# achiever04/face-recognition-platform

Measured on AMD Instinct MI355X. Metric: faces/sec (detect+embed+match) on 1080p @ 100k gallery, higher is better.
Workload: dtype f16; 1 GPU; 32x1080x1920 BGR frames per GPU per step resident in HBM, host results out every step, 2 batches in flight per GPU (one handle = one stream each, used round-robin), forced K=10 faces/frame, 100000-identity fp16 gallery, FRPDet detector fp16 + ArcFace IResNet-100 fp16 (synthetic seeded weights); batch_frames=32, faces_per_frame=10, gallery=100000, streams=1, lanes=2, lane_warmup_steps=20

## Files before the change

### face-recognition-platform_amd/csrc/aux_kernels.hip

```cpp
#include <hip/hip_runtime.h>
#include <stdint.h>
#include "frp_internal.h"

namespace frp {

typedef _Float16 half8 __attribute__((ext_vector_type(8)));

__global__ __launch_bounds__(256) void preprocess_kernel(const uint8_t* __restrict__ src, int B, int H, int W,
                                                         long row_stride, long frame_stride,
                                                         _Float16* __restrict__ out, int Hc, int Wc, int rgb_in) {
    const long total = (long)B * Hc * Wc;
    for (long i = (long)blockIdx.x * blockDim.x + threadIdx.x; i < total; i += (long)gridDim.x * blockDim.x) {
        const int x = (int)(i % Wc);
        const long r = i / Wc;
        const int y = (int)(r % Hc);
        const int b = (int)(r / Hc);
        float c0 = 0.f, c1 = 0.f, c2 = 0.f;
        if (y < H && x < W) {
            const uint8_t* p = src + b * frame_stride + y * row_stride + 3L * x;
            c0 = (float)p[0]; c1 = (float)p[1]; c2 = (float)p[2];
        }
        const float r_ = rgb_in ? c0 : c2, g_ = c1, b_ = rgb_in ? c2 : c0;
        half8 v;
        v[0] = (_Float16)((r_ - 127.5f) * (1.0f / 128.0f));
// ... 299 lines not shown
    return hipGetLastError();
}

hipError_t launch_mfma_peak(const _Float16* src, float* dst, int blocks, int iters, hipStream_t stream) {
    hipLaunchKernelGGL(mfma_peak_kernel, dim3(blocks), dim3(256), 0, stream, src, dst, iters);
    return hipGetLastError();
}

hipError_t launch_fill_random_f16(_Float16* p, long n, unsigned seed, float scale, hipStream_t stream) {
    if (n <= 0) return hipSuccess;
    hipLaunchKernelGGL(fill_random_f16_kernel, dim3(4096), dim3(256), 0, stream, p, n, seed, scale);
    return hipGetLastError();
}
#endif

__global__ __launch_bounds__(256) void tensor_hash_kernel(const uint4* __restrict__ src, long n16, unsigned long long* __restrict__ slot) {
    unsigned long long acc = 0;
    for (long i = (long)blockIdx.x * blockDim.x + threadIdx.x; i < n16; i += (long)gridDim.x * blockDim.x) {
        const uint4 v = src[i];
        unsigned long long a = ((unsigned long long)v.x << 32 | v.y) ^ 0x9e3779b97f4a7c15ull * (unsigned long long)(i + 1);
        unsigned long long b = ((unsigned long long)v.z << 32 | v.w) + 0xc2b2ae3d27d4eb4full * (unsigned long long)(i + 1);
        a ^= a >> 29; a *= 0xbf58476d1ce4e5b9ull; a ^= a >> 32;
        b ^= b >> 31; b *= 0x94d049bb133111ebull; b ^= b >> 29;
        acc += a + (b << 1 | b >> 63);
    }
#pragma unroll
    for (int o = 32; o; o >>= 1) acc += __shfl_xor(acc, o);
    if ((threadIdx.x & 63) == 0) atomicAdd(slot, acc);
}
hipError_t launch_tensor_hash(const void* src, size_t bytes, unsigned long long* slot, hipStream_t stream) {
    const long n16 = (long)(bytes / 16);
    if (n16 <= 0) return hipSuccess;
    hipLaunchKernelGGL(tensor_hash_kernel, dim3(1024), dim3(256), 0, stream, (const uint4*)src, n16, slot);
    return hipGetLastError();
}

}
```

### face-recognition-platform_amd/csrc/frp_api.cpp

```cpp
#include <hip/hip_runtime.h>

#include <algorithm>
#include <cmath>
#include <cstdio>
#include <cstdlib>
#include <cstring>
#include <mutex>
#include <string>
#include <vector>
#include <thread>
#include <atomic>

#include "frp.h"
#include "frp_blob.h"
#include "frp_internal.h"
#include "frp_handle.h"
#include "jpeg_host.h"

using namespace frp;

#define FRP_WINO_MIN_FACES 128
Switches frp::read_switches() {
    auto set = [](const char* n) { return getenv(n) ? 1 : 0; };
    const char *sm = getenv("FRP_SMALL_M"), *wm = getenv("FRP_WINO_MIN_FACES");
    Switches s{};
    s.small_m = !sm ? 0 : (sm[0] == '0' ? -1 : 1);
    s.wino_min_faces = wm ? atoi(wm) : FRP_WINO_MIN_FACES;
    s.s2 = set("FRP_S2"); s.host_count = set("FRP_HOST_COUNT"); s.match_v1 = set("FRP_MATCH_V1");
    s.no_fused_stem12 = set("FRP_NO_FUSED_STEM12"); s.no_fused_stem = set("FRP_NO_FUSED_STEM");
    s.no_emb_stem = set("FRP_NO_EMB_STEM"); s.no_stem_fuse = set("FRP_NO_STEM_FUSE");
    s.no_wino = set("FRP_NO_WINO"); s.no_kconcat = set("FRP_NO_KCONCAT");
    return s;
}

const ProcessSwitches& frp::process_switches() {
    static const ProcessSwitches s = [] {
        const char* jh = getenv("FRP_JPEG_DEVICE_HUFFMAN");
        return ProcessSwitches{getenv("FRP_NO_GRAPH") != nullptr, getenv("FRP_C64_ALL") != nullptr, !jh ? 0 : (jh[0] == '0' ? -1 : 1)};
    }();
    return s;
// ... 1025 lines not shown
int frp_debug_det_hashes(frp_handle* h, int32_t enable, uint64_t* out64) {
    if (!h) return FRP_ERR_INVALID;
    Guard g(h);
    if (enable) {
        FRPCHK(ensure(h, h->det_hashes, 64 * 8));
        h->det_hash_on = true;
    } else h->det_hash_on = false;
    if (out64) {
        if (!h->det_hashes.p) return fail(h, FRP_ERR_INVALID, "hashes were never enabled");
        HIPCHK(h, hipMemcpyAsync(out64, h->det_hashes.p, 64 * 8, hipMemcpyDeviceToHost, h->stream));
        HIPCHK(h, hipStreamSynchronize(h->stream));
    }
    return FRP_OK;
}

int frp_debug_det_prefix(frp_handle* h, int32_t n_ops, void* out_f16, int64_t out_bytes, int32_t* th, int32_t* tw, int32_t* tc) {
    if (!h) return FRP_ERR_INVALID;
    Guard g(h);
    if (!h->have_weights) return fail(h, FRP_ERR_NO_WEIGHTS, "no weights loaded");
    if (h->rB <= 0) return fail(h, FRP_ERR_INVALID, "no resident frames (call frp_upload_frames)");
    if (n_ops <= 0 || n_ops > (int)h->det.ops.size()) return fail(h, FRP_ERR_INVALID, "op count out of range");
    const int B = h->rB, Hc = h->canvas_h, Wc = h->canvas_w;
    const Switches sw = read_switches();
    const bool fused = h->det.det_stem && !sw.no_fused_stem;
    if (!fused) return fail(h, FRP_ERR_INVALID, "prefix runs need the fused stem");
    if (n_ops == 1 && h->det.det_stem12 && (Hc % 4) == 0 && (Wc % 4) == 0 && !sw.no_fused_stem12)
        return fail(h, FRP_ERR_INVALID, "op 0 has no tensor while both stems run as one kernel: set FRP_NO_FUSED_STEM12 to read the stem1 map");
    FRPCHK(plan_net(h, h->det, B, Hc, Wc, fused));
    StemParams sp{};
    sp.frames = h->det_scaled ? (const uint8_t*)h->scaled.p : (const uint8_t*)h->frames.p;
// ... 279 lines not shown
```

### face-recognition-platform_amd/csrc/frp_internal.h

```cpp
#pragma once
#include <hip/hip_runtime.h>
#include <stdint.h>
#include <type_traits>

#define FRP_ACT_NONE 0
#define FRP_ACT_RELU 1
#define FRP_ACT_PRELU 2
#define FRP_FLAG_BORDER_BIAS 1
#define FRP_FLAG_OUT_F32 2
#define FRP_FLAG_RES_UP2 4
#define FRP_FLAG_FLATTEN 8
#define FRP_FLAG_F8 32
#define FRP_FLAG_OUT_FP8 64
#define FRP_CHIP_PIX (112 * 112)
#ifndef FRP_MAX_FACES_CAP
#define FRP_MAX_FACES_CAP 128
#endif

#include "jpeg_host.h"

namespace frp {

struct Switches {
    int small_m;
    int s2;
    int no_fused_stem12;
    int no_fused_stem;
    int no_emb_stem;
    int no_stem_fuse;
    int wino_min_faces;
    int host_count;
    int match_v1;
    int no_wino;
    int no_kconcat;
};
static_assert(std::has_unique_object_representations_v<Switches>, "run_net keys captured graphs by the bytes of a Switches");
Switches read_switches();

struct ProcessSwitches {
    bool no_graph;
    bool c64_all;
    int jpeg_device_huffman;
};
const ProcessSwitches& process_switches();

struct ConvParams {
    const _Float16* x;
    const _Float16* w;
    const float* bias;
// ... 148 lines not shown

struct JpegHuffParams {
    const uint8_t* scan;
    const uint32_t* int_off;
    const JpegHuffTableDev* tables;
    int16_t* coef;
    int32_t* err;
    long coef_per_image;
    int B, n_int, ri;
    int mcus_x, mcus_y, components;
    int hs[3], vs[3], bx[3];
    long comp_off[3];
};
hipError_t launch_jpeg_huffman(const JpegHuffParams& p, hipStream_t stream);

hipError_t launch_tensor_hash(const void* src, size_t bytes, unsigned long long* slot, hipStream_t stream);
hipError_t launch_resize_u8(const uint8_t* src, int B, int H, int W, uint8_t* dst, int Hs, int Ws, hipStream_t stream);

struct AlignParams {
    const uint8_t* frames;
    int B, H, W;
    long row_stride, frame_stride;
    const float* kps;
    const int32_t* counts;
    int max_faces;
    const int32_t* face_slot;
    int n_faces;
    int rgb_in;
    _Float16* chips;
    const int32_t* n_dev;
};
// ... 72 lines not shown
```

### face-recognition-platform_amd/csrc/net_program.cpp

```cpp
#include "net_program.h"

#include <algorithm>
#include <cmath>
#include <cstdio>
#include <cstring>

#include "frp_handle.h"

namespace frp {

static float fp8_e4m3_value(unsigned char c) {
    const int e = (c >> 3) & 0xF, m = c & 7;
    float v;
    if (e == 15 && m == 7) v = 0.f;
    else if (e == 0) v = std::ldexp((float)m / 8.0f, -6);
    else v = std::ldexp(1.0f + (float)m / 8.0f, e - 7);
    return (c & 0x80) ? -v : v;
}

uint16_t f32_to_f16_bits(float f) {
    uint32_t x;
    memcpy(&x, &f, 4);
    const uint32_t sign = (x >> 16) & 0x8000u;
    x &= 0x7fffffffu;
// ... 247 lines not shown
}

void analyse_net(Net& net) {
    const int n = (int)net.ops.size();
    net.det_stem = stem_fusable(net);
    net.det_stem12 = stem12_fusable(net);
    net.fc_op = n && (net.ops[n - 1].flags & FRP_FLAG_OUT_F32) ? n - 1 : -1;
    net.next_launch.assign(n, -1);
    for (int i = n - 1, nx = -1; i >= 0; --i) {
        net.next_launch[i] = nx;
        if (!net.kc_skip[i]) nx = i;
    }
    net.emb_stem = net.fuse_ok = net.fuse_even_only = false;
    net.fuse_op = -1;
    if (n) analyse_emb_stem(net);
}

}

int load_program(frp_handle* h, const frp_blob_header& hd, const unsigned char* blob, size_t bytes, const Switches& sw,
                 std::vector<unsigned char>& image) {
    Net &det = h->det, &emb = h->emb;
    det.is_det = true;
    FRPCHK(parse_net(h, blob, bytes, hd.det_ops_offset, hd.n_det_ops, hd.n_det_bufs, hd.det_in_buf, hd.det_in_ch, hd.data_bytes, det));
    FRPCHK(parse_net(h, blob, bytes, hd.emb_ops_offset, hd.n_emb_ops, hd.n_emb_bufs, hd.emb_in_buf, hd.emb_in_ch, hd.data_bytes, emb));
    for (int l = 0; l < 3; ++l)
        if (hd.det_head_buf[l] >= hd.n_det_bufs) return fail(h, FRP_ERR_BLOB, "head buffer id out of range");
    if (hd.emb_out_buf >= hd.n_emb_bufs) return fail(h, FRP_ERR_BLOB, "embedding buffer id out of range");
    image.assign(blob + hd.data_offset, blob + hd.data_offset + hd.data_bytes);
    for (Net* net : {&det, &emb}) {
        const size_t n_ops = net->ops.size();
        net->wino_off.assign(n_ops, -1);
// ... 47 lines not shown
    for (int i = 0; i < net.n_bufs; ++i)
        if (need[i]) FRPCHK(ensure(h, net.bufs[i], need[i]));
    return FRP_OK;
}

namespace {

struct Pass {
    frp_handle* h;
    const Switches& sw;
    Net& net;
    int batch, H, W;
    const StemParams* stem;
    const int32_t* n_dev;
    bool allow_wino;
    const char* weights() const { return (const char*)h->wdata.p; }
};

struct FusedStem {
    bool on = false;
    EmbStemParams p{};
};

int launched(frp_handle* h, hipError_t e, const char* what) {
    return e == hipSuccess ? FRP_OK : fail(h, FRP_ERR_HIP, std::string(what) + ": " + hipGetErrorString(e));
}

int run_det_stems(const Pass& ps, PassEffects& fx, size_t& next) {
    frp_handle* h = ps.h;
    const Net& net = ps.net;
    const StemParams& st = *ps.stem;
    const char* wbase = ps.weights();
    if (net.ops.empty()) return FRP_OK;
    const frp_conv_op& a = net.ops[0];
    if (net.det_stem12 && (st.Hc % 4) == 0 && (st.Wc % 4) == 0 && !ps.sw.no_fused_stem12) {
        const frp_conv_op& b = net.ops[1];
        Stem12Params sp{};
        sp.frames = st.frames; sp.B = st.B; sp.H = st.H; sp.W = st.W;
        sp.row_stride = st.row_stride; sp.frame_stride = st.frame_stride;
        sp.Hc = st.Hc; sp.Wc = st.Wc; sp.Ho1 = st.Hc / 2; sp.Wo1 = st.Wc / 2; sp.Ho2 = st.Hc / 4; sp.Wo2 = st.Wc / 4;
        sp.rgb_in = st.rgb_in;
        sp.w1 = (const _Float16*)(wbase + a.w_off); sp.bias1 = (const float*)(wbase + a.bias_off);
        sp.w2 = (const _Float16*)(wbase + b.w_off); sp.bias2 = (const float*)(wbase + b.bias_off);
        sp.out = (_Float16*)net.bufs[b.out_buf].p;
        FRPCHK(launched(h, launch_stem12_u8(sp, h->stream), "launch_stem12_u8"));
        fx.dims[a.out_buf] = {sp.Ho1, sp.Wo1, 32, false};
        fx.dims[b.out_buf] = {sp.Ho2, sp.Wo2, 64, false};
        fx.flops += 2.0 * ps.batch * sp.Ho1 * sp.Wo1 * 9.0 * 3 * 32 + 2.0 * ps.batch * sp.Ho2 * sp.Wo2 * 9.0 * 32 * 64;
        fx.launches += 1;
        next = 2;
        if (!h->det_hash_on) return FRP_OK;
        return launched(h, launch_tensor_hash(sp.out, (size_t)ps.batch * sp.Ho2 * sp.Wo2 * 64 * 2, (unsigned long long*)h->det_hashes.p + 1, h->stream),
                        "tensor_hash");
    }
    StemParams sp = st;
    sp.w = (const _Float16*)(wbase + a.w_off);
    sp.bias = (const float*)(wbase + a.bias_off);
    sp.out = (_Float16*)net.bufs[a.out_buf].p;
    FRPCHK(launched(h, launch_stem_u8(sp, h->stream), "launch_stem_u8"));
    fx.dims[a.out_buf] = {sp.Ho, sp.Wo, 32, false};
    fx.flops += 2.0 * ps.batch * sp.Ho * sp.Wo * 9.0 * 3 * 32;
    fx.launches += 1;
    next = 1;
    return FRP_OK;
}

int run_emb_stem(const Pass& ps, PassEffects& fx, size_t& next, FusedStem& fused) {
    const Net& net = ps.net;
    if (!net.emb_stem || ps.sw.no_emb_stem) return FRP_OK;
    const frp_conv_op& a = net.ops[0];
    const char* wbase = ps.weights();
    EmbStemParams ep{};
    ep.x = (const _Float16*)net.bufs[a.in_buf].p;
    ep.M = ps.batch; ep.H = ps.H; ep.W = ps.W;
    ep.w = (const _Float16*)(wbase + a.w_off);
    ep.bias = (const float*)(wbase + a.bias_off);
    ep.slope = (const float*)(wbase + a.slope_off);
    ep.out = (_Float16*)net.bufs[a.out_buf].p;
    ep.n_dev = ps.n_dev;
    fused.on = net.fuse_ok && !ps.sw.no_stem_fuse && ps.sw.small_m <= 0 && conv3x3_c64_fuses_stem(ps.batch, ps.H, ps.W, ps.h->n_cu);
    if (fused.on) {
        fused.p = ep;
    } else {
        FRPCHK(launched(ps.h, launch_emb_stem(ep, ps.h->stream), "launch_emb_stem"));
        fx.launches += 1;
    }
    fx.dims[a.out_buf] = {ps.H, ps.W, 64, false};
    fx.flops += 2.0 * ps.batch * ps.H * ps.W * 9.0 * 3 * 64;
    next = 1;
    return FRP_OK;
}

ConvParams conv_params_for(const Pass& ps, size_t i, const TensorDims& in, const std::vector<TensorDims>& d, const FusedStem& fused) {
// ... 27 lines not shown
        p.flags |= FRP_FLAG_F8;
        p.wscale = (const float*)(wbase + op.w_off + (welems + 15) / 16 * 16);
        p.in_scale = op.in_scale;
    }
    if (net.kc_src[i] >= 0) {
        const frp_conv_op& sc = net.ops[net.kc_src[i]];
        p.x2 = (const _Float16*)net.bufs[sc.in_buf].p;
        p.Cin2 = sc.cin;
        p.w = (const _Float16*)(wbase + net.kc_w_off[i]);
        p.bias = (const float*)(wbase + net.kc_bias_off[i]);
        p.res = nullptr;
    }
    if (op.flags & FRP_OPFLAG_OUT_FP8) p.flags |= FRP_FLAG_OUT_FP8;
    if (op.out2_buf >= 0) p.out2 = net.bufs[op.out2_buf].p;
    if ((op.flags & FRP_OPFLAG_OUT_FP8) || op.out2_buf >= 0) p.out_scale = op.out_scale;
    const int nx = net.next_launch[i];
    if (nx < 0) return p;
    const frp_conv_op& no = net.ops[nx];
    if (net.kc_src[nx] >= 0) {
        p.pf_ptr = wbase + net.kc_w_off[nx];
        p.pf_bytes = (unsigned)((size_t)no.cout * (9 * (size_t)no.cin + net.ops[net.kc_src[nx]].cin) * 2);
    } else if (ps.allow_wino && net.wino_off[nx] >= 0) {
        p.pf_ptr = wbase + net.wino_off[nx];
        p.pf_bytes = (unsigned)std::min<size_t>(conv3x3_wino_image_bytes(no.cin, no.cout), 0x7fffffffu);
    } else {
        const size_t es = (no.flags & FRP_OPFLAG_FP8_MFMA) ? 1 : 2;
        p.pf_ptr = wbase + no.w_off;
        p.pf_bytes = (unsigned)std::min<size_t>((size_t)no.cout * no.ksize * no.ksize * no.cin * es, 0x7fffffffu);
    }
    return p;
// ... 8 lines not shown
    p.ksplit = ps.n_dev ? -1 : ks;
    p.out = h->splitk_ws.p;
    fc.ksplit = p.ksplit;
    fc.bias = p.bias;
    fc.ktot = op.ksize * op.ksize * op.cin;
}

void charge(const frp_conv_op& op, const TensorDims& out, int batch, PassEffects& fx) {
    const int cin_r = op.real_ch & 0xffff, cout_r = (op.real_ch >> 16) & 0xffff;
    const double fl = 2.0 * batch * out.h * out.w * (double)op.ksize * op.ksize * (cin_r ? cin_r : op.cin) * (cout_r ? cout_r : op.cout);
    fx.flops += fl;
    fx.launches += 1;
    if (op.flags & FRP_OPFLAG_FP8_MFMA) { fx.f8_flops += fl; fx.f8_launches += 1; }
}

int walk(const Pass& ps, PassEffects& fx) {
    frp_handle* h = ps.h;
    const Net& net = ps.net;
    fx = PassEffects();
    std::vector<TensorDims>& d = fx.dims;
    d.assign(net.n_bufs, TensorDims());
    d[net.in_buf] = {ps.H, ps.W, net.in_ch, false};
    const bool hashing = net.is_det && h->det_hash_on;
    if (hashing) HIPCHK(h, hipMemsetAsync(h->det_hashes.p, 0, 64 * 8, h->stream));
    size_t i = 0;
    FusedStem fused;
    if (ps.stem) FRPCHK(run_det_stems(ps, fx, i));
    else FRPCHK(run_emb_stem(ps, fx, i, fused));
    size_t end = net.ops.size();
    if (net.is_det && h->det_op_limit >= 0) end = std::min(end, (size_t)h->det_op_limit);
    for (; i < end; ++i) {
        const frp_conv_op& op = net.ops[i];
        const TensorDims in = flat_input(d[op.in_buf], op), out = conv_out_dims(in, op);
        if (net.kc_skip[i]) {
            set_out_dims(d, op, out);
            fx.flops += 2.0 * ps.batch * out.h * out.w * (double)op.cin * op.cout;
            continue;
        }
        ConvParams p = conv_params_for(ps, i, in, d, fused);
        if ((int)i == net.fc_op) pick_fc_splitk(ps, op, in, out, p, fx.fc);
        FRPCHK(launched(h, launch_conv(p, h->stream), "launch_conv"));
        set_out_dims(d, op, out);
        if (hashing && i < 64 && !ps.n_dev)
            FRPCHK(launched(h, launch_tensor_hash(net.bufs[op.out_buf].p, (size_t)ps.batch * out.h * out.w * out.c * (out.f32 ? 4 : 2),
                                                  (unsigned long long*)h->det_hashes.p + i, h->stream), "tensor_hash"));
        charge(op, out, ps.batch, fx);
    }
    return FRP_OK;
}

std::string graph_key(const Pass& ps) {
    char kb[512];
    int len = snprintf(kb, sizeof kb, "%c|%d|%d|%d|%d|%p|%p|", ps.net.is_det ? 'd' : 'e', ps.batch, ps.H, ps.W, (int)ps.allow_wino, (const void*)ps.n_dev,
                       (const void*)ps.h->wdata.p);
    if (const StemParams* stem = ps.stem; stem && len > 0 && len < (int)sizeof kb)
        len += snprintf(kb + len, sizeof kb - len, "%p|%d|%d|%d|%ld|%ld|%d|%d|%d", (const void*)stem->frames, stem->B, stem->H, stem->W, stem->row_stride,
                        stem->frame_stride, stem->Hc, stem->Wc, stem->rgb_in);
    if (len <= 0 || len >= (int)sizeof kb) return std::string();
    return std::string(kb, len) + std::string(reinterpret_cast<const char*>(&ps.sw), sizeof ps.sw);
}

int launch_or_replay(const Pass& ps, PassEffects& fx) {
    frp_handle* h = ps.h;
    if (process_switches().no_graph || h->det_hash_on || h->det_op_limit >= 0) return walk(ps, fx);
    const std::string key = graph_key(ps);
    if (key.empty()) return walk(ps, fx);
    for (size_t i = 0; i < h->graphs.size(); ++i) {
        NetGraph& g = h->graphs[i];
        if (g.key != key) continue;
        if (g.epoch != h->alloc_epoch) {
            (void)hipGraphExecDestroy(g.exec);
            h->graphs.erase(h->graphs.begin() + i);
// ... 76 lines not shown
```

### face-recognition-platform_amd/csrc/net_program.h

```cpp
#pragma once
#include <string>
#include <vector>

#include "frp_blob.h"
#include "frp_internal.h"

struct frp_handle;

namespace frp {

struct DevBuf {
    void* p = nullptr;
    size_t cap = 0;
};

struct TensorDims {
    int h = 0, w = 0, c = 0;
    bool f32 = false;
    bool f8 = false;
};

struct Net {
    std::vector<frp_conv_op> ops;
    int n_bufs = 0;
// ... 1 lines not shown
    bool is_det = false;
    std::vector<DevBuf> bufs;
    std::vector<TensorDims> dims;
    std::vector<int64_t> wino_off;
    std::vector<int> kc_skip;
    std::vector<int> kc_src;
    std::vector<int64_t> kc_w_off, kc_bias_off;
    bool det_stem = false;
    bool det_stem12 = false;
    bool emb_stem = false;
    int fuse_op = -1;
    bool fuse_ok = false;
    bool fuse_even_only = false;
    int fc_op = -1;
    std::vector<int> next_launch;
};

struct FcSplitK {
    int ksplit = 0, ktot = 0;
    const float* bias = nullptr;
};

struct PassEffects {
    double flops = 0, f8_flops = 0;
    int64_t launches = 0, f8_launches = 0;
    FcSplitK fc;
    std::vector<TensorDims> dims;
};

struct NetGraph {
    std::string key;
// ... 21 lines not shown
```

### face-recognition-platform_amd/native.py

```python
from __future__ import annotations

import ctypes as C
import os
import threading
from typing import Optional, Sequence, Tuple

import numpy as np

_HERE = os.path.dirname(os.path.abspath(__file__))
os.environ.setdefault("GPU_MAX_HW_QUEUES", "8")

LIB_PATH = os.environ.get("FRP_LIB") or os.path.join(_HERE, "libfrp.so")

EMB_DIM = 512
CHIP = 112
MAX_FACES_CAP = 128
MAX_TOPK = 64
FLAG_FORCED_K, FLAG_RGB, FLAG_NO_MATCH, FLAG_WITHIN = 1, 2, 4, 8
F32, F16, F64 = 0, 1, 2
QUALITY_TILE_H, QUALITY_TILE_W = 32, 64

ABI_SYMBOLS = [
    "frp_create", "frp_destroy", "frp_last_error", "frp_version", "frp_load_weights",
    "frp_gallery_set", "frp_gallery_set_device", "frp_gallery_reserve", "frp_gallery_commit", "frp_gallery_cancel", "frp_gallery_device_ptr", "frp_gallery_update_row", "frp_gallery_remove_row",
    "frp_jpeg_info_get", "frp_jpeg_coefficients", "frp_upload_jpeg_async", "frp_debug_jpeg_device_batches", "frp_debug_graph_replays",
    "frp_dist_unique_id", "frp_dist_init", "frp_dist_destroy", "frp_gallery_allgather",
    "frp_gallery_size", "frp_gallery_get", "frp_gallery_exact", "frp_gallery_distances", "frp_gallery_get_exact",
    "frp_process_frames", "frp_upload_frames", "frp_process_resident", "frp_fetch_results", "frp_synchronize",
    "frp_host_alloc", "frp_host_free", "frp_upload_frames_async", "frp_swap_frames",
    "frp_detect", "frp_detect_resident", "frp_get_det_source", "frp_finish_faces", "frp_get_head_map", "frp_debug_det_prefix", "frp_debug_det_hashes", "frp_decode_heads", "frp_align", "frp_embed_aligned", "frp_embed_faces",
    "frp_match", "frp_match_scores", "frp_match_within", "frp_set_within", "frp_fetch_within", "frp_face_quality", "frp_conv2d_nhwc", "frp_conv2d_f8", "frp_get_counters", "frp_reset_counters", "frp_set_profile",
]


class FrpConfig(C.Structure):
    _fields_ = [("struct_size", C.c_int32), ("max_batch", C.c_int32), ("max_faces", C.c_int32),
                ("max_h", C.c_int32), ("max_w", C.c_int32), ("profile", C.c_int32), ("reserved", C.c_int32 * 10)]


class FrpCounters(C.Structure):
    _fields_ = [("struct_size", C.c_int32), ("calls", C.c_int32), ("frames", C.c_int64), ("faces", C.c_int64),
                ("ms_h2d", C.c_double), ("ms_preprocess", C.c_double), ("ms_det_conv", C.c_double),
                ("ms_decode", C.c_double), ("ms_align", C.c_double), ("ms_emb_conv", C.c_double),
                ("ms_l2norm", C.c_double), ("ms_match", C.c_double), ("ms_d2h", C.c_double), ("ms_total", C.c_double),
                ("det_conv_flops", C.c_double), ("emb_conv_flops", C.c_double),
# ... 35 lines not shown

def jpeg_coefficients(data: bytes):
    info = jpeg_info(data)
    if info is None:
        raise FrpError(-1, "not a baseline JPEG the decoder covers")
    n = sum(info["mcus_x"] * info["h_samp"][c] * info["mcus_y"] * info["v_samp"][c] * 64 for c in range(info["components"]))
    coef = np.zeros(n, np.int16)
    q = np.zeros((3, 64), np.uint16)
    ji = JpegInfo()
    ptr, keep = _byte_ptr(data)
    rc = load_library().frp_jpeg_coefficients(ptr, len(data), _ptr(coef), n, _ptr(q), C.byref(ji))
    del keep
    if rc != 0:
        raise FrpError(rc, "corrupt JPEG scan data")
    return info, coef, q


class FrpError(RuntimeError):
    def __init__(self, code: int, msg: str):
        super().__init__(f"frp error {code}: {msg}")
        self.code = code


_lib = None


def kernel_source_hash() -> str:
    import glob
    import hashlib
    h = hashlib.sha256()
# ... 53 lines not shown
    lib.frp_detect.argtypes = [vp, vp, i32, i32, i32, i64, i32, f32, f32, u32, vp, vp, vp, vp, vp]
    lib.frp_detect_resident.argtypes = [vp, i32, i32, i32, i32, f32, f32, u32, vp, vp, vp, vp, vp]
    lib.frp_get_det_source.argtypes = [vp, vp, i64, C.POINTER(i32), C.POINTER(i32)]
    lib.frp_finish_faces.argtypes = [vp, i32, vp, vp, vp, vp, i32, u32, vp, vp, vp]
    lib.frp_get_head_map.argtypes = [vp, i32, vp, i64, C.POINTER(i32), C.POINTER(i32)]
    lib.frp_debug_jpeg_device_batches.argtypes = [vp]
    lib.frp_debug_jpeg_device_batches.restype = C.c_int64
    lib.frp_debug_graph_replays.argtypes = [vp]
    lib.frp_debug_graph_replays.restype = C.c_int64
    lib.frp_dist_unique_id.argtypes = [vp]
    lib.frp_dist_init.argtypes = [vp, vp, i32, i32]
    lib.frp_dist_destroy.argtypes = [vp]
    lib.frp_gallery_allgather.argtypes = [vp, vp, i64, i32, i64]
    lib.frp_debug_det_prefix.argtypes = [vp, i32, vp, i64, C.POINTER(i32), C.POINTER(i32), C.POINTER(i32)]
    lib.frp_debug_det_hashes.argtypes = [vp, i32, vp]
    lib.frp_decode_heads.argtypes = [vp, vp, vp, vp, i32, i32, i32, i32, f32, f32, u32, vp, vp, vp, vp, vp]
    lib.frp_align.argtypes = [vp, vp, i32, i32, i64, vp, i32, u32, vp]
    lib.frp_embed_aligned.argtypes = [vp, vp, i32, vp]
    lib.frp_embed_faces.argtypes = [vp, vp, i32, i32, i64, vp, i32, u32, vp]
    lib.frp_match.argtypes = [vp, vp, i32, i32, vp, vp]
    lib.frp_match_scores.argtypes = [vp, vp, i32, vp, i64]
    if hasattr(lib, "frp_match_within"):
        lib.frp_match_within.argtypes = [vp, vp, i32, f32, i32, vp, vp, vp]
        lib.frp_set_within.argtypes = [vp, f32, i32]
        lib.frp_fetch_within.argtypes = [vp, i32, i32, i32, vp, vp, vp]
    if hasattr(lib, "frp_face_quality"):
        lib.frp_face_quality.argtypes = [vp, vp, i32, u32, vp]
    lib.frp_conv2d_nhwc.argtypes = [vp, vp, i32, i32, i32, i32, vp, i32, i32, i32, vp, vp, vp, i32, i32, i32, i32, vp]
    lib.frp_conv2d_f8.argtypes = [vp, vp, i32, i32, i32, i32, vp, i32, vp, vp, vp, vp, i32, i32, f32, f32, vp, vp]
    if hasattr(lib, "frp_kstep_lab"):
# ... 478 lines not shown
```

### include/frp.h

```cpp
#ifndef FRP_H
#define FRP_H

#include <stddef.h>
#include <stdint.h>

#ifdef __cplusplus
extern "C" {
#endif

#define FRP_EMB_DIM 512
#define FRP_CHIP 112
#define FRP_KPS 5
#define FRP_MAX_FACES_CAP 128
#define FRP_MAX_TOPK 64

typedef enum frp_status {
    FRP_OK = 0,
    FRP_ERR_INVALID = -1,
    FRP_ERR_HIP = -2,
    FRP_ERR_NO_WEIGHTS = -3,
    FRP_ERR_NO_GALLERY = -4,
    FRP_ERR_BLOB = -5,
    FRP_ERR_OOM = -6
} frp_status;
// ... 91 lines not shown
int frp_dist_destroy(frp_handle* h);
int frp_gallery_allgather(frp_handle* h, const void* shard, int64_t shard_rows, int32_t dtype, int64_t n_total);

int frp_detect(frp_handle* h, const uint8_t* bgr, int32_t B, int32_t H, int32_t W, int64_t row_stride,
               int32_t max_faces, float det_thresh, float nms_iou, uint32_t flags,
               float* boxes, float* kps, float* scores, int32_t* counts, int32_t* anchor_idx);
int frp_detect_resident(frp_handle* h, int32_t B, int32_t det_h, int32_t det_w, int32_t max_faces, float det_thresh, float nms_iou,
                        uint32_t flags, float* boxes, float* kps, float* scores, int32_t* counts, int32_t* anchor_idx);
int frp_get_det_source(frp_handle* h, uint8_t* out, int64_t out_bytes, int32_t* hs, int32_t* ws);
int frp_finish_faces(frp_handle* h, int32_t B, const float* boxes, const float* kps, const float* scores, const int32_t* counts,
                     int32_t max_faces, uint32_t flags, float* emb, int32_t* match_idx, float* match_cos);

int frp_get_head_map(frp_handle* h, int32_t level, void* out_f16, int64_t out_bytes, int32_t* hl, int32_t* wl);
int frp_debug_det_prefix(frp_handle* h, int32_t n_ops, void* out_f16, int64_t out_bytes, int32_t* th, int32_t* tw, int32_t* tc);
int frp_debug_det_hashes(frp_handle* h, int32_t enable, uint64_t* out64);
int frp_decode_heads(frp_handle* h, const void* head8, const void* head16, const void* head32,
                     int32_t B, int32_t canvas_h, int32_t canvas_w, int32_t max_faces, float det_thresh, float nms_iou,
                     uint32_t flags, float* boxes, float* kps, float* scores, int32_t* counts, int32_t* anchor_idx);
int frp_align(frp_handle* h, const uint8_t* bgr, int32_t H, int32_t W, int64_t row_stride,
              const float* kps, int32_t M, uint32_t flags, void* chips_f16);
int frp_embed_aligned(frp_handle* h, const uint8_t* chips, int32_t M, float* emb);
int frp_embed_faces(frp_handle* h, const uint8_t* bgr, int32_t H, int32_t W, int64_t row_stride,
                    const float* kps, int32_t M, uint32_t flags, float* emb);
int frp_match(frp_handle* h, const float* q, int32_t M, int32_t topk, int32_t* idx, float* cos);
int frp_match_scores(frp_handle* h, const float* q, int32_t M, float* cos_all, int64_t n_cols);
int frp_match_within(frp_handle* h, const float* q, int32_t M, float min_cos, int32_t cap, int32_t* idx, float* cos, int32_t* n_hits);

int frp_face_quality(frp_handle* h, const int32_t* rects, int32_t n, uint32_t flags, int64_t* sums);

int frp_conv2d_nhwc(frp_handle* h, const void* x, int32_t N, int32_t H, int32_t W, int32_t Cin,
// ... 17 lines not shown
```

Baseline: 27220 faces/s.

## Run front detector layers in frame groups so activations stay cache-resident

Finds the leading run of frame-local conv ops whose activation maps are large, then executes that run group-by-group over frames instead of layer-by-layer over the whole batch. The group size is chosen so live activations per group fit a byte budget (about the last-level cache size), with some preference for groups that fill the CUs evenly. The aim is to keep intermediate maps from spilling to HBM between layers. In exchange it issues more, smaller kernel launches with lower occupancy per launch, and the graph key now includes the plan. A hash offset parameter and a debug plan API are added.

New measurement: 26630 faces/s. 0.978x the previous value.

```diff
diff --git a/face-recognition-platform_amd/csrc/aux_kernels.hip b/face-recognition-platform_amd/csrc/aux_kernels.hip
--- a/face-recognition-platform_amd/csrc/aux_kernels.hip
+++ b/face-recognition-platform_amd/csrc/aux_kernels.hip
@@ -337,10 +337,11 @@
 }
 #endif
 
-__global__ __launch_bounds__(256) void tensor_hash_kernel(const uint4* __restrict__ src, long n16, unsigned long long* __restrict__ slot) {
+__global__ __launch_bounds__(256) void tensor_hash_kernel(const uint4* __restrict__ src, long n16, long first16, unsigned long long* __restrict__ slot) {
     unsigned long long acc = 0;
-    for (long i = (long)blockIdx.x * blockDim.x + threadIdx.x; i < n16; i += (long)gridDim.x * blockDim.x) {
-        const uint4 v = src[i];
+    for (long j = (long)blockIdx.x * blockDim.x + threadIdx.x; j < n16; j += (long)gridDim.x * blockDim.x) {
+        const uint4 v = src[j];
+        const long i = j + first16;
         unsigned long long a = ((unsigned long long)v.x << 32 | v.y) ^ 0x9e3779b97f4a7c15ull * (unsigned long long)(i + 1);
         unsigned long long b = ((unsigned long long)v.z << 32 | v.w) + 0xc2b2ae3d27d4eb4full * (unsigned long long)(i + 1);
         a ^= a >> 29; a *= 0xbf58476d1ce4e5b9ull; a ^= a >> 32;
@@ -351,11 +352,11 @@
     for (int o = 32; o; o >>= 1) acc += __shfl_xor(acc, o);
     if ((threadIdx.x & 63) == 0) atomicAdd(slot, acc);
 }
-hipError_t launch_tensor_hash(const void* src, size_t bytes, unsigned long long* slot, hipStream_t stream) {
+hipError_t launch_tensor_hash(const void* src, size_t bytes, unsigned long long* slot, hipStream_t stream, size_t first_byte) {
     const long n16 = (long)(bytes / 16);
     if (n16 <= 0) return hipSuccess;
-    hipLaunchKernelGGL(tensor_hash_kernel, dim3(1024), dim3(256), 0, stream, (const uint4*)src, n16, slot);
-    return hipGetLastError();
-}
-
-}
+    hipLaunchKernelGGL(tensor_hash_kernel, dim3(1024), dim3(256), 0, stream, (const uint4*)src, n16, (long)(first_byte / 16), slot);
+    return hipGetLastError();
+}
+
+}
diff --git a/face-recognition-platform_amd/csrc/frp_api.cpp b/face-recognition-platform_amd/csrc/frp_api.cpp
--- a/face-recognition-platform_amd/csrc/frp_api.cpp
+++ b/face-recognition-platform_amd/csrc/frp_api.cpp
@@ -22,8 +22,9 @@
 #define FRP_WINO_MIN_FACES 128
 Switches frp::read_switches() {
     auto set = [](const char* n) { return getenv(n) ? 1 : 0; };
-    const char *sm = getenv("FRP_SMALL_M"), *wm = getenv("FRP_WINO_MIN_FACES");
+    const char *sm = getenv("FRP_SMALL_M"), *wm = getenv("FRP_WINO_MIN_FACES"), *fg = getenv("FRP_FRONT_GROUP");
     Switches s{};
+    s.front_group = fg ? std::max(0, atoi(fg)) : -1;
     s.small_m = !sm ? 0 : (sm[0] == '0' ? -1 : 1);
     s.wino_min_faces = wm ? atoi(wm) : FRP_WINO_MIN_FACES;
     s.s2 = set("FRP_S2"); s.host_count = set("FRP_HOST_COUNT"); s.match_v1 = set("FRP_MATCH_V1");
@@ -1079,6 +1080,30 @@
     return FRP_OK;
 }
 
+int frp_debug_front_plan(const void* blob, size_t bytes, int32_t which, int32_t batch, int32_t H, int32_t W, int32_t n_cu, int32_t* first,
+                         int32_t* last, int32_t* group) {
+    if (!blob || bytes < sizeof(frp_blob_header) || batch <= 0 || H <= 0 || W <= 0 || (which != 0 && which != 1)) return FRP_ERR_INVALID;
+    frp_blob_header hd;
+    memcpy(&hd, blob, sizeof(hd));
+    if (memcmp(hd.magic, FRP_BLOB_MAGIC, 8) != 0 || hd.version != FRP_BLOB_VERSION || hd.header_bytes != sizeof(frp_blob_header)) return FRP_ERR_BLOB;
+    if (hd.data_offset > bytes || hd.data_bytes > bytes - hd.data_offset) return FRP_ERR_BLOB;
+    const Switches sw = read_switches();
+    frp_handle tmp;
+    std::vector<unsigned char> image;
+    FRPCHK(load_program(&tmp, hd, (const unsigned char*)blob, bytes, sw, image));
+    const Net& net = which == 0 ? tmp.det : tmp.emb;
+    FrontCall c;
+    c.batch = batch; c.H = H; c.W = W; c.n_cu = n_cu > 0 ? n_cu : 256;
+    c.force = sw.front_group;
+    c.u8_input = which == 0 && net.det_stem && !sw.no_fused_stem;
+    c.stem12 = c.u8_input && net.det_stem12 && (H % 4) == 0 && (W % 4) == 0 && !sw.no_fused_stem12;
+    const FrontRun run = find_front_run(net, c);
+    if (first) *first = run.first;
+    if (last) *last = run.last;
+    if (group) *group = run.group;
+    return FRP_OK;
+}
+
 int frp_debug_det_prefix(frp_handle* h, int32_t n_ops, void* out_f16, int64_t out_bytes, int32_t* th, int32_t* tw, int32_t* tc) {
     if (!h) return FRP_ERR_INVALID;
     Guard g(h);
diff --git a/face-recognition-platform_amd/csrc/frp_internal.h b/face-recognition-platform_amd/csrc/frp_internal.h
--- a/face-recognition-platform_amd/csrc/frp_internal.h
+++ b/face-recognition-platform_amd/csrc/frp_internal.h
@@ -33,6 +33,7 @@
     int match_v1;
     int no_wino;
     int no_kconcat;
+    int front_group;
 };
 static_assert(std::has_unique_object_representations_v<Switches>, "run_net keys captured graphs by the bytes of a Switches");
 Switches read_switches();
@@ -211,7 +212,7 @@
 };
 hipError_t launch_jpeg_huffman(const JpegHuffParams& p, hipStream_t stream);
 
-hipError_t launch_tensor_hash(const void* src, size_t bytes, unsigned long long* slot, hipStream_t stream);
+hipError_t launch_tensor_hash(const void* src, size_t bytes, unsigned long long* slot, hipStream_t stream, size_t first_byte = 0);
 hipError_t launch_resize_u8(const uint8_t* src, int B, int H, int W, uint8_t* dst, int Hs, int Ws, hipStream_t stream);
 
 struct AlignParams {
diff --git a/face-recognition-platform_amd/csrc/net_program.cpp b/face-recognition-platform_amd/csrc/net_program.cpp
--- a/face-recognition-platform_amd/csrc/net_program.cpp
+++ b/face-recognition-platform_amd/csrc/net_program.cpp
@@ -285,8 +285,118 @@
     net.emb_stem = net.fuse_ok = net.fuse_even_only = false;
     net.fuse_op = -1;
     if (n) analyse_emb_stem(net);
-}
-
+    net.frame_local.assign(n, 0);
+    for (int i = 0; i < n; ++i) {
+        const frp_conv_op& op = net.ops[i];
+        const int heavy = FRP_FLAG_OUT_F32 | FRP_FLAG_FLATTEN | FRP_OPFLAG_W_FP8 | FRP_OPFLAG_FP8_MFMA | FRP_OPFLAG_OUT_FP8;
+        net.frame_local[i] = !(op.flags & heavy) && op.out2_buf < 0 && net.wino_off[i] < 0;
+    }
+}
+
+}
+
+int pick_front_group(int batch, size_t live_per_frame, long tiles_per_frame, int n_cu, size_t budget) {
+    if (batch <= 1 || live_per_frame == 0) return 0;
+    const size_t gmax = std::max<size_t>(budget / live_per_frame, 1);
+    if (gmax >= (size_t)batch) return 0;
+    const long cu = n_cu > 0 ? n_cu : 256;
+    auto fill = [&](long g) {
+        const long t = g * std::max(tiles_per_frame, 1L);
+        return (double)t / (double)((t + cu - 1) / cu * cu);
+    };
+    long best = (long)gmax;
+    for (long g = (long)gmax - 1; g > (long)gmax / 2; --g)
+        if (fill(g) > fill(best) + 0.005) best = g;
+    return (int)best;
+}
+
+FrontRun find_front_run(const Net& net, const FrontCall& c, size_t map_bytes, size_t budget) {
+    FrontRun none;
+    const int n = (int)net.ops.size(), end = c.end >= 0 ? std::min(c.end, n) : n;
+    if (c.force == 0 || c.batch <= 1 || end <= 0 || (int)net.frame_local.size() != n) return none;
+    struct Touch { size_t in = 0, res = 0, x2 = 0, out = 0; int res_buf = -1, x2_buf = -1; long in_pix = 0, out_pix = 0; };
+    std::vector<Touch> t(n);
+    std::vector<TensorDims> d(net.n_bufs);
+    d[net.in_buf] = {c.H, c.W, net.in_ch, false};
+    auto bytes = [](const TensorDims& x) { return (size_t)x.h * x.w * x.c * (x.f32 ? 4 : x.f8 ? 1 : 2); };
+    size_t largest = 0;
+    for (int i = 0; i < end; ++i) {
+        const frp_conv_op& op = net.ops[i];
+        if (d[op.in_buf].c == 0) return none;
+        const TensorDims in = flat_input(d[op.in_buf], op), out = conv_out_dims(in, op);
+        const bool no_in = i == 0 ? c.u8_input : (i == 1 && c.stem12);
+        const bool no_out = i == 0 && c.stem12;
+        t[i].in = no_in ? 0 : bytes(in);
+        t[i].out = no_out ? 0 : bytes(out);
+        t[i].in_pix = (long)in.h * in.w;
+        t[i].out_pix = (long)out.h * out.w;
+        if (net.kc_src[i] >= 0) {
+            t[i].x2_buf = net.ops[net.kc_src[i]].in_buf;
+            t[i].x2 = bytes(d[t[i].x2_buf]);
+        } else if (op.res_buf >= 0) {
+            t[i].res_buf = op.res_buf;
+            t[i].res = bytes(d[op.res_buf]);
+        }
+        if (net.kc_skip[i]) t[i].res = t[i].out = 0;
+        set_out_dims(d, op, out);
+        for (size_t b : {t[i].in, t[i].res, t[i].x2, t[i].out}) largest = std::max(largest, b);
+    }
+    auto big = [&](size_t b) { return b && (c.force > 0 ? b == largest : b * (size_t)c.batch > map_bytes); };
+    auto touches_big = [&](int i) {
+        if (i == 0 && c.stem12 && end > 1) i = 1;
+        return big(t[i].in) || big(t[i].res) || big(t[i].x2) || big(t[i].out);
+    };
+    int first = -1, last = -1;
+    std::vector<size_t> held(net.n_bufs, 0);
+    for (int i = 0; i < end; ++i) {
+        const frp_conv_op& op = net.ops[i];
+        const bool in_run = net.frame_local[i] && (net.kc_skip[i] ? first >= 0 && big(t[i].in) : touches_big(i));
+        if (!in_run) {
+            if (first >= 0) break;
+            continue;
+        }
+        bool ok = true;
+        if (!net.kc_skip[i]) {
+            const size_t reads[3] = {t[i].in, t[i].res, t[i].x2};
+            const int read_bufs[3] = {op.in_buf, t[i].res_buf, t[i].x2_buf};
+            for (int k = 0; k < 3; ++k)
+                if (read_bufs[k] >= 0 && reads[k] && !held[read_bufs[k]]) held[read_bufs[k]] = reads[k];
+            ok = !t[i].out || !held[op.out_buf] || t[i].out <= held[op.out_buf];
+            if (ok && t[i].out) held[op.out_buf] = t[i].out;
+        }
+        if (!ok) break;
+        if (first < 0) first = i;
+        if (!net.kc_skip[i]) last = i;
+    }
+    if (first < 0 || last < 0) return none;
+    if (net.emb_stem && net.fuse_op >= 0 && (first == 0) != (net.fuse_op >= first && net.fuse_op <= last)) return none;
+    FrontRun run;
+    run.first = first;
+    run.last = last;
+    for (int i = first; i <= last; ++i) {
+        if (net.kc_skip[i]) continue;
+        const frp_conv_op& op = net.ops[i];
+        size_t live = t[i].out;
+        for (int b : {op.in_buf, t[i].res_buf, t[i].x2_buf}) {
+            if (b < 0) continue;
+            bool from_run = false;
+            for (int q = first; q < i; ++q) from_run |= !net.kc_skip[q] && t[q].out && net.ops[q].out_buf == b;
+            if (!from_run) live += b == op.in_buf ? t[i].in : b == t[i].res_buf ? t[i].res : t[i].x2;
+        }
+        for (int q = first; q < i; ++q) {
+            if (net.kc_skip[q] || !t[q].out) continue;
+            bool read_later = false;
+            for (int r = i; r <= last && !read_later; ++r)
+                read_later = !net.kc_skip[r] && (net.ops[r].in_buf == net.ops[q].out_buf || t[r].res_buf == net.ops[q].out_buf ||
+                                                 t[r].x2_buf == net.ops[q].out_buf);
+            if (read_later) live += t[q].out;
+        }
+        run.live_per_frame = std::max(run.live_per_frame, live);
+        const long pixels = std::max(big(t[i].in) ? t[i].in_pix : 0, big(t[i].out) ? t[i].out_pix : 0);
+        run.tiles_per_frame = std::max(run.tiles_per_frame, (pixels + 255) / 256);
+    }
+    run.group = c.force > 0 ? std::min(c.force, c.batch) : pick_front_group(c.batch, run.live_per_frame, run.tiles_per_frame, c.n_cu, budget);
+    return run;
 }
 
 int load_program(frp_handle* h, const frp_blob_header& hd, const unsigned char* blob, size_t bytes, const Switches& sw,
@@ -364,8 +474,16 @@
     const StemParams* stem;
     const int32_t* n_dev;
     bool allow_wino;
+    int frame0 = 0;
     const char* weights() const { return (const char*)h->wdata.p; }
 };
+
+template <class T> T* frames_in(T* p, int frames, size_t per_frame, size_t elem = sizeof(T)) {
+    return p ? (T*)((const char*)p + (size_t)frames * per_frame * elem) : p;
+}
+template <> void* frames_in<void>(void* p, int frames, size_t per_frame, size_t elem) {
+    return p ? (char*)p + (size_t)frames * per_frame * elem : p;
+}
 
 struct FusedStem {
     bool on = false;
@@ -386,13 +504,14 @@
     if (net.det_stem12 && (st.Hc % 4) == 0 && (st.Wc % 4) == 0 && !ps.sw.no_fused_stem12) {
         const frp_conv_op& b = net.ops[1];
         Stem12Params sp{};
-        sp.frames = st.frames; sp.B = st.B; sp.H = st.H; sp.W = st.W;
+        sp.frames = st.frames + (long)ps.frame0 * st.frame_stride; sp.B = ps.batch; sp.H = st.H; sp.W = st.W;
         sp.row_stride = st.row_stride; sp.frame_stride = st.frame_stride;
         sp.Hc = st.Hc; sp.Wc = st.Wc; sp.Ho1 = st.Hc / 2; sp.Wo1 = st.Wc / 2; sp.Ho2 = st.Hc / 4; sp.Wo2 = st.Wc / 4;
         sp.rgb_in = st.rgb_in;
         sp.w1 = (const _Float16*)(wbase + a.w_off); sp.bias1 = (const float*)(wbase + a.bias_off);
         sp.w2 = (const _Float16*)(wbase + b.w_off); sp.bias2 = (const float*)(wbase + b.bias_off);
-        sp.out = (_Float16*)net.bufs[b.out_buf].p;
+        const size_t per_frame = (size_t)sp.Ho2 * sp.Wo2 * 64;
+        sp.out = frames_in((_Float16*)net.bufs[b.out_buf].p, ps.frame0, per_frame);
         FRPCHK(launched(h, launch_stem12_u8(sp, h->stream), "launch_stem12_u8"));
         fx.dims[a.out_buf] = {sp.Ho1, sp.Wo1, 32, false};
         fx.dims[b.out_buf] = {sp.Ho2, sp.Wo2, 64, false};
@@ -400,13 +519,15 @@
         fx.launches += 1;
         next = 2;
         if (!h->det_hash_on) return FRP_OK;
-        return launched(h, launch_tensor_hash(sp.out, (size_t)ps.batch * sp.Ho2 * sp.Wo2 * 64 * 2, (unsigned long long*)h->det_hashes.p + 1, h->stream),
-                        "tensor_hash");
+        return launched(h, launch_tensor_hash(sp.out, ps.batch * per_frame * 2, (unsigned long long*)h->det_hashes.p + 1, h->stream,
+                                              ps.frame0 * per_frame * 2), "tensor_hash");
     }
     StemParams sp = st;
+    sp.frames = st.frames + (long)ps.frame0 * st.frame_stride;
+    sp.B = ps.batch;
     sp.w = (const _Float16*)(wbase + a.w_off);
     sp.bias = (const float*)(wbase + a.bias_off);
-    sp.out = (_Float16*)net.bufs[a.out_buf].p;
+    sp.out = frames_in((_Float16*)net.bufs[a.out_buf].p, ps.frame0, (size_t)sp.Ho * sp.Wo * 32);
     FRPCHK(launched(h, launch_stem_u8(sp, h->stream), "launch_stem_u8"));
     fx.dims[a.out_buf] = {sp.Ho, sp.Wo, 32, false};
     fx.flops += 2.0 * ps.batch * sp.Ho * sp.Wo * 9.0 * 3 * 32;
@@ -421,12 +542,12 @@
     const frp_conv_op& a = net.ops[0];
     const char* wbase = ps.weights();
     EmbStemParams ep{};
-    ep.x = (const _Float16*)net.bufs[a.in_buf].p;
+    ep.x = frames_in((const _Float16*)net.bufs[a.in_buf].p, ps.frame0, (size_t)ps.H * ps.W * 8);
     ep.M = ps.batch; ep.H = ps.H; ep.W = ps.W;
     ep.w = (const _Float16*)(wbase + a.w_off);
     ep.bias = (const float*)(wbase + a.bias_off);
     ep.slope = (const float*)(wbase + a.slope_off);
-    ep.out = (_Float16*)net.bufs[a.out_buf].p;
+    ep.out = frames_in((_Float16*)net.bufs[a.out_buf].p, ps.frame0, (size_t)ps.H * ps.W * 64);
     ep.n_dev = ps.n_dev;
     fused.on = net.fuse_ok && !ps.sw.no_stem_fuse && ps.sw.small_m <= 0 && conv3x3_c64_fuses_stem(ps.batch, ps.H, ps.W, ps.h->n_cu);
     if (fused.on) {
@@ -484,6 +605,15 @@
     if (op.flags & FRP_OPFLAG_OUT_FP8) p.flags |= FRP_FLAG_OUT_FP8;
     if (op.out2_buf >= 0) p.out2 = net.bufs[op.out2_buf].p;
     if ((op.flags & FRP_OPFLAG_OUT_FP8) || op.out2_buf >= 0) p.out_scale = op.out_scale;
+    if (ps.frame0) {
+        const TensorDims out = conv_out_dims(in, op);
+        const size_t out_px = (size_t)out.h * out.w;
+        p.x = frames_in(p.x, ps.frame0, (size_t)in.h * in.w * in.c, in.f8 ? 1 : 2);
+        p.res = frames_in(p.res, ps.frame0, (op.flags & FRP_FLAG_RES_UP2) ? (size_t)p.Hr * p.Wr * op.cout : out_px * op.cout);
+        p.out = frames_in(p.out, ps.frame0, out_px * out.c, out.f32 ? 4 : out.f8 ? 1 : 2);
+        p.out2 = frames_in(p.out2, ps.frame0, out_px * out.c, 1);
+        if (p.x2) p.x2 = frames_in(p.x2, ps.frame0, (size_t)in.h * in.w * p.Cin2);
+    }
     const int nx = net.next_launch[i];
     if (nx < 0) return p;
     const frp_conv_op& no = net.ops[nx];
@@ -522,6 +652,49 @@
     if (op.flags & FRP_OPFLAG_FP8_MFMA) { fx.f8_flops += fl; fx.f8_launches += 1; }
 }
 
+int walk_ops(const Pass& ps, PassEffects& fx, size_t i, size_t end, const FusedStem& fused) {
+    frp_handle* h = ps.h;
+    const Net& net = ps.net;
+    std::vector<TensorDims>& d = fx.dims;
+    const bool hashing = net.is_det && h->det_hash_on;
+    for (; i < end; ++i) {
+        const frp_conv_op& op = net.ops[i];
+        const TensorDims in = flat_input(d[op.in_buf], op), out = conv_out_dims(in, op);
+        if (net.kc_skip[i]) {
+            set_out_dims(d, op, out);
+            fx.flops += 2.0 * ps.batch * out.h * out.w * (double)op.cin * op.cout;
+            continue;
+        }
+        ConvParams p = conv_params_for(ps, i, in, d, fused);
+        if ((int)i == net.fc_op) pick_fc_splitk(ps, op, in, out, p, fx.fc);
+        FRPCHK(launched(h, launch_conv(p, h->stream), "launch_conv"));
+        set_out_dims(d, op, out);
+        if (hashing && i < 64 && !ps.n_dev) {
+            const size_t per_frame = (size_t)out.h * out.w * out.c * (out.f32 ? 4 : 2);
+            FRPCHK(launched(h, launch_tensor_hash(frames_in(net.bufs[op.out_buf].p, ps.frame0, per_frame, 1), ps.batch * per_frame, (unsigned long long*)h->det_hashes.p + i, h->stream,
+                                                  ps.frame0 * per_frame), "tensor_hash"));
+        }
+        charge(op, out, ps.batch, fx);
+    }
+    return FRP_OK;
+}
+
+size_t pass_end(const Pass& ps) {
+    const size_t n = ps.net.ops.size();
+    return ps.net.is_det && ps.h->det_op_limit >= 0 ? std::min(n, (size_t)ps.h->det_op_limit) : n;
+}
+
+FrontRun front_run_of(const Pass& ps) {
+    if (ps.n_dev) return FrontRun();
+    FrontCall c;
+    c.batch = ps.batch; c.H = ps.H; c.W = ps.W; c.n_cu = ps.h->n_cu;
+    c.force = ps.sw.front_group;
+    c.u8_input = ps.stem != nullptr;
+    c.stem12 = ps.stem && ps.net.det_stem12 && (ps.stem->Hc % 4) == 0 && (ps.stem->Wc % 4) == 0 && !ps.sw.no_fused_stem12;
+    c.end = (int)pass_end(ps);
+    return find_front_run(ps.net, c);
+}
+
 int walk(const Pass& ps, PassEffects& fx) {
     frp_handle* h = ps.h;
     const Net& net = ps.net;
@@ -531,30 +704,29 @@
     d[net.in_buf] = {ps.H, ps.W, net.in_ch, false};
     const bool hashing = net.is_det && h->det_hash_on;
     if (hashing) HIPCHK(h, hipMemsetAsync(h->det_hashes.p, 0, 64 * 8, h->stream));
+    const size_t end = pass_end(ps);
+    const FrontRun run = front_run_of(ps);
+    auto stems = [&](const Pass& q, size_t& next, FusedStem& fused) {
+        return q.stem ? run_det_stems(q, fx, next) : run_emb_stem(q, fx, next, fused);
+    };
     size_t i = 0;
     FusedStem fused;
-    if (ps.stem) FRPCHK(run_det_stems(ps, fx, i));
-    else FRPCHK(run_emb_stem(ps, fx, i, fused));
-    size_t end = net.ops.size();
-    if (net.is_det && h->det_op_limit >= 0) end = std::min(end, (size_t)h->det_op_limit);
-    for (; i < end; ++i) {
-        const frp_conv_op& op = net.ops[i];
-        const TensorDims in = flat_input(d[op.in_buf], op), out = conv_out_dims(in, op);
-        if (net.kc_skip[i]) {
-            set_out_dims(d, op, out);
-            fx.flops += 2.0 * ps.batch * out.h * out.w * (double)op.cin * op.cout;
-            continue;
-        }
-        ConvParams p = conv_params_for(ps, i, in, d, fused);
-        if ((int)i == net.fc_op) pick_fc_splitk(ps, op, in, out, p, fx.fc);
-        FRPCHK(launched(h, launch_conv(p, h->stream), "launch_conv"));
-        set_out_dims(d, op, out);
-        if (hashing && i < 64 && !ps.n_dev)
-            FRPCHK(launched(h, launch_tensor_hash(net.bufs[op.out_buf].p, (size_t)ps.batch * out.h * out.w * out.c * (out.f32 ? 4 : 2),
-                                                  (unsigned long long*)h->det_hashes.p + i, h->stream), "tensor_hash"));
-        charge(op, out, ps.batch, fx);
-    }
-    return FRP_OK;
+    if (run.group <= 0 || run.first > 0) FRPCHK(stems(ps, i, fused));
+    if (run.group > 0) {
+        const size_t start = std::max(i, (size_t)run.first), stop = std::max(start, (size_t)run.last + 1);
+        FRPCHK(walk_ops(ps, fx, i, start, fused));
+        for (int g0 = 0; g0 < ps.batch; g0 += run.group) {
+            Pass sl = ps;
+            sl.frame0 = g0;
+            sl.batch = std::min(run.group, ps.batch - g0);
+            size_t j = start;
+            FusedStem fs = fused;
+            if (run.first == 0) FRPCHK(stems(sl, j, fs));
+            FRPCHK(walk_ops(sl, fx, j, stop, fs));
+        }
+        i = stop;
+    }
+    return walk_ops(ps, fx, i, end, fused);
 }
 
 std::string graph_key(const Pass& ps) {
@@ -564,6 +736,10 @@
     if (const StemParams* stem = ps.stem; stem && len > 0 && len < (int)sizeof kb)
         len += snprintf(kb + len, sizeof kb - len, "%p|%d|%d|%d|%ld|%ld|%d|%d|%d", (const void*)stem->frames, stem->B, stem->H, stem->W, stem->row_stride,
                         stem->frame_stride, stem->Hc, stem->Wc, stem->rgb_in);
+    if (len > 0 && len < (int)sizeof kb) {
+        const FrontRun run = front_run_of(ps);
+        len += snprintf(kb + len, sizeof kb - len, "|g%d:%d:%d|", run.first, run.last, run.group);
+    }
     if (len <= 0 || len >= (int)sizeof kb) return std::string();
     return std::string(kb, len) + std::string(reinterpret_cast<const char*>(&ps.sw), sizeof ps.sw);
 }
diff --git a/face-recognition-platform_amd/csrc/net_program.h b/face-recognition-platform_amd/csrc/net_program.h
--- a/face-recognition-platform_amd/csrc/net_program.h
+++ b/face-recognition-platform_amd/csrc/net_program.h
@@ -39,7 +39,26 @@
     bool fuse_even_only = false;
     int fc_op = -1;
     std::vector<int> next_launch;
+    std::vector<int> frame_local;
 };
+
+constexpr size_t FRONT_MAP_BYTES = (size_t)256 << 20;
+constexpr size_t FRONT_GROUP_BUDGET = (size_t)208 << 20;
+struct FrontRun {
+    int first = -1, last = -1;
+    int group = 0;
+    size_t live_per_frame = 0;
+    long tiles_per_frame = 0;
+};
+struct FrontCall {
+    int batch = 0, H = 0, W = 0, n_cu = 256;
+    int force = -1;
+    bool u8_input = false;
+    bool stem12 = false;
+    int end = -1;
+};
+FrontRun find_front_run(const Net& net, const FrontCall& c, size_t map_bytes = FRONT_MAP_BYTES, size_t budget = FRONT_GROUP_BUDGET);
+int pick_front_group(int batch, size_t live_per_frame, long tiles_per_frame, int n_cu, size_t budget);
 
 struct FcSplitK {
     int ksplit = 0, ktot = 0;
diff --git a/face-recognition-platform_amd/native.py b/face-recognition-platform_amd/native.py
--- a/face-recognition-platform_amd/native.py
+++ b/face-recognition-platform_amd/native.py
@@ -28,7 +28,7 @@
     "frp_gallery_size", "frp_gallery_get", "frp_gallery_exact", "frp_gallery_distances", "frp_gallery_get_exact",
     "frp_process_frames", "frp_upload_frames", "frp_process_resident", "frp_fetch_results", "frp_synchronize",
     "frp_host_alloc", "frp_host_free", "frp_upload_frames_async", "frp_swap_frames",
-    "frp_detect", "frp_detect_resident", "frp_get_det_source", "frp_finish_faces", "frp_get_head_map", "frp_debug_det_prefix", "frp_debug_det_hashes", "frp_decode_heads", "frp_align", "frp_embed_aligned", "frp_embed_faces",
+    "frp_detect", "frp_detect_resident", "frp_get_det_source", "frp_finish_faces", "frp_get_head_map", "frp_debug_det_prefix", "frp_debug_det_hashes", "frp_debug_front_plan", "frp_decode_heads", "frp_align", "frp_embed_aligned", "frp_embed_faces",
     "frp_match", "frp_match_scores", "frp_match_within", "frp_set_within", "frp_fetch_within", "frp_face_quality", "frp_conv2d_nhwc", "frp_conv2d_f8", "frp_get_counters", "frp_reset_counters", "frp_set_profile",
 ]
 
@@ -94,6 +94,17 @@
     if rc != 0:
         raise FrpError(rc, "corrupt JPEG scan data")
     return info, coef, q
+
+
+def front_plan(blob: bytes, which: str, batch: int, H: int, W: int, n_cu: int = 256):
+    first, last, group = C.c_int32(-1), C.c_int32(-1), C.c_int32(0)
+    ptr, keep = _byte_ptr(blob)
+    rc = load_library().frp_debug_front_plan(ptr, len(blob), {"det": 0, "emb": 1}[which], batch, H, W, n_cu,
+                                             C.byref(first), C.byref(last), C.byref(group))
+    del keep
+    if rc != 0:
+        raise FrpError(rc, "front plan: bad blob or arguments")
+    return first.value, last.value, group.value
 
 
 class FrpError(RuntimeError):
@@ -177,6 +188,8 @@
     lib.frp_gallery_allgather.argtypes = [vp, vp, i64, i32, i64]
     lib.frp_debug_det_prefix.argtypes = [vp, i32, vp, i64, C.POINTER(i32), C.POINTER(i32), C.POINTER(i32)]
     lib.frp_debug_det_hashes.argtypes = [vp, i32, vp]
+    if hasattr(lib, "frp_debug_front_plan"):
+        lib.frp_debug_front_plan.argtypes = [vp, C.c_size_t, i32, i32, i32, i32, i32, C.POINTER(i32), C.POINTER(i32), C.POINTER(i32)]
     lib.frp_decode_heads.argtypes = [vp, vp, vp, vp, i32, i32, i32, i32, f32, f32, u32, vp, vp, vp, vp, vp]
     lib.frp_align.argtypes = [vp, vp, i32, i32, i64, vp, i32, u32, vp]
     lib.frp_embed_aligned.argtypes = [vp, vp, i32, vp]
diff --git a/include/frp.h b/include/frp.h
--- a/include/frp.h
+++ b/include/frp.h
@@ -129,6 +129,8 @@
 int frp_get_head_map(frp_handle* h, int32_t level, void* out_f16, int64_t out_bytes, int32_t* hl, int32_t* wl);
 int frp_debug_det_prefix(frp_handle* h, int32_t n_ops, void* out_f16, int64_t out_bytes, int32_t* th, int32_t* tw, int32_t* tc);
 int frp_debug_det_hashes(frp_handle* h, int32_t enable, uint64_t* out64);
+int frp_debug_front_plan(const void* blob, size_t bytes, int32_t which, int32_t batch, int32_t H, int32_t W, int32_t n_cu, int32_t* first,
+                         int32_t* last, int32_t* group);
 int frp_decode_heads(frp_handle* h, const void* head8, const void* head16, const void* head32,
                      int32_t B, int32_t canvas_h, int32_t canvas_w, int32_t max_faces, float det_thresh, float nms_iou,
                      uint32_t flags, float* boxes, float* kps, float* scores, int32_t* counts, int32_t* anchor_idx);
```
